# NVlabs/FasterViT

Measured on AMD Instinct MI355X. Metric: images/sec FasterViT-0 224x224 inference, bs=256/GPU, higher is better.
Workload: dtype f16; 1 GPU; faster_vit_0_224 inference, 224x224, batch 256/GPU, synthetic weights (tests/synth.py init family); global_batch=256, parallelism=dp1 (independent shards, no data-path collective), hat_operands=f16, streams=1

## Files before the change

fastervit_amd/csrc/fvit_conv.hip:

```cpp
#include "fvit_common.h"

namespace fvit {

namespace {

constexpr int BK = 64;

struct ConvParams {
    const void* in;
    const void* w;
    const float* bias;
    const void* res;
    void* out;
    const void* zeros;
    int B, Hi, Wi, Cin, Cout, Ho, Wo, stride, act;
    int M, tiles_m, tiles_n;
    int ablate;
    int wterms;
    const void* in_lo;
    const void* res_lo;
    void* out_lo;
    float* out_f32;
    int px;
    int cv, kd;
    float inv_cv;
};

__device__ __forceinline__ int swz_x(int r) { return (r >> 1) & 7; }
__device__ __forceinline__ int swz_w(int r) { return ((0x78 >> (2 * ((r >> 4) & 3))) & 3) | ((r & 2) << 1); }

__device__ __forceinline__ void glds16(const void* gsrc, char* lds_dst) {
    __builtin_amdgcn_global_load_lds((const __attribute__((address_space(1))) void*)gsrc,
                                     (__attribute__((address_space(3))) void*)lds_dst, 16, 0, 0);
}

template <int V> struct IntTag { static constexpr int value = V; };
template <typename F>
__device__ __forceinline__ void dispatch_epilogue(int act, bool has_res, F&& body) {
    if (has_res) {
        if (act == 0) body(IntTag<0>{}, IntTag<1>{});
        else if (act == 1) body(IntTag<1>{}, IntTag<1>{});
        else body(IntTag<2>{}, IntTag<1>{});
    } else {
        if (act == 0) body(IntTag<0>{}, IntTag<0>{});
        else if (act == 1) body(IntTag<1>{}, IntTag<0>{});
        else body(IntTag<2>{}, IntTag<0>{});
    }
}

constexpr int PATCH_H = 8, PATCH_W = 16, PHALO_W = PATCH_W + 2, PHALO_ROWS = (PATCH_H + 2) * PHALO_W;
constexpr int PHALO_PIECES = (PHALO_ROWS + 7) / 8;
constexpr int PHALO_BYTES = PHALO_PIECES * 1024;

template <typename T, int WM, int WN, int NI, bool PX = false, bool DENSE = false, bool HALO = false>
__global__ __launch_bounds__(256, 2) void conv3x3_kernel(ConvParams p) {
    typedef typename Op16<T>::v8 v8;
    static_assert(!HALO || (WM == 2 && WN == 2 && !DENSE), "halo form: 8 x 16 patches on the 2 x 2 wave grid, classic weight layout");
    constexpr int BM = 64 * WM, BN = 16 * NI * WN;
    constexpr int X_BYTES = HALO ? PHALO_BYTES : BM * BK * 2, W_BYTES = BN * BK * 2;
    constexpr int XP = BM / 8 / 4;
    constexpr int HP = (PHALO_PIECES + 3) / 4;
    constexpr int WPIECES = BN / 8;
    constexpr int WP = (WPIECES + 3) / 4;
    static_assert(2 * (X_BYTES + W_BYTES) <= 80 * 1024, "two workgroups per CU");
    __shared__ __attribute__((aligned(16))) char smem[2 * (X_BYTES + W_BYTES)];

    const int tid = threadIdx.x;
    const int lane = tid & 63;
    const int wave = __builtin_amdgcn_readfirstlane(tid >> 6);
    const int wm = wave / WN, wn = wave - wm * WN;

    const int nblk = gridDim.x, b = blockIdx.x;
    const int q = nblk >> 3, rr = nblk & 7, xcd = b & 7, idx = b >> 3;
    const int v = (xcd < rr ? xcd * (q + 1) : rr * (q + 1) + (xcd - rr) * q) + idx;
    const int tm = v / p.tiles_n, tn = v - tm * p.tiles_n;
    const int m0 = tm * BM, n0 = tn * BN;

    const T* __restrict__ In = (const T*)p.in;
    const T* __restrict__ W = (const T*)p.w;
    const T* __restrict__ Z = (const T*)p.zeros;
    const int ldw = DENSE ? p.wterms * p.kd * BK : p.wterms * 9 * p.Cin;

    f4 acc[NI][4];
#pragma unroll
    for (int i = 0; i < NI; ++i)
#pragma unroll
        for (int j = 0; j < 4; ++j) acc[i][j] = (f4){0.f, 0.f, 0.f, 0.f};

    const int g = lane >> 4, s = lane & 15;
    int bimg = 0, y0 = 0, x0 = 0;
    if constexpr (HALO) {
        const int tpx = (p.Wo + PATCH_W - 1) / PATCH_W, tpy = (p.Ho + PATCH_H - 1) / PATCH_H;
        bimg = tm / (tpy * tpx);
        const int rem = tm - bimg * (tpy * tpx);
        const int ty = rem / tpx;
        y0 = ty * PATCH_H;
        x0 = (rem - ty * tpx) * PATCH_W;
    }
    if constexpr (HALO) {
        int hoff[HP];
        int hvalid = 0;
        int hchunk[HP];
#pragma unroll
        for (int i = 0; i < HP; ++i) {
            const int piece = wave + 4 * i;
            const int r = piece * 8 + (lane >> 3);
            const int hy = r / PHALO_W, hx = r - hy * PHALO_W;
            const int iy = y0 - 1 + hy, ix = x0 - 1 + hx;
            const int chunk = ((lane & 7) ^ swz_x(r)) * 8;
            hchunk[i] = chunk;
            const bool ok = piece < PHALO_PIECES && r < PHALO_ROWS && iy >= 0 && iy < p.Hi && ix >= 0 && ix < p.Wi;
            if (ok) hvalid |= 1 << i;
            hoff[i] = ok ? ((bimg * p.Hi + iy) * p.Wi + ix) * p.Cin + chunk : 0;
        }
        const int ncc = p.Cin / BK;
        const int kpb_hi = p.wterms * 9;
        const int nblk_hi = ncc, nblk_all = ncc * ((PX && p.in_lo) ? 2 : 1);
        const int nk = nblk_hi * kpb_hi + (nblk_all - nblk_hi) * 9;
        const T* const InLo = (PX && p.in_lo) ? (const T*)p.in_lo : In;
        auto stage_halo = [&](int blk, char* xbuf) {
            const bool lo = blk >= nblk_hi;
            const T* const plane = lo ? InLo : In;
            const int c0 = (lo ? blk - nblk_hi : blk) * BK;
#pragma unroll
            for (int i = 0; i < HP; ++i) {
                const int piece = wave + 4 * i;
                if (piece < PHALO_PIECES) {
                    const T* src = ((hvalid >> i) & 1) ? plane + (hoff[i] + c0) : Z + hchunk[i];
                    glds16(src, xbuf + piece * 1024);
                }
            }
        };
        auto stage_w = [&](int blk, int kin, char* wbuf) {
            const bool lo = blk >= nblk_hi;
            const int c0 = (lo ? blk - nblk_hi : blk) * BK;
            const int col = kin * p.Cin + c0;
#pragma unroll
            for (int i = 0; i < WP; ++i) {
                const int piece = wave * WP + i;
                if (piece < WPIECES) {
                    const int r = piece * 8 + (lane >> 3);
                    const int c = (lane & 7) ^ swz_w(r);
                    glds16(W + (size_t)min(n0 + r, p.Cout - 1) * ldw + col + c * 8, wbuf + piece * 1024);
                }
            }
        };
        char* const wring = smem + 2 * X_BYTES;
        stage_halo(0, smem);
        stage_w(0, 0, wring);
        int rbase[4], wrow[NI];
#pragma unroll
        for (int i = 0; i < 4; ++i) rbase[i] = (wm * 4 + i) * PHALO_W + s;
#pragma unroll
        for (int i = 0; i < NI; ++i) wrow[i] = wn * 16 * NI + (s >> 2) * 4 * NI + i * 4 + (s & 3);
        int blk = 0, kin = 0, kpb = kpb_hi, hb = 0;
        for (int kt = 0; kt < nk; ++kt) {
            asm volatile("s_waitcnt vmcnt(0)" ::: "memory");
            __syncthreads();
            const int cur = kt & 1;
            int nblk_ = blk, nkin = kin + 1;
            if (nkin == kpb) { nblk_ = blk + 1; nkin = 0; }
            if (kt + 1 < nk) stage_w(nblk_, nkin, wring + (cur ^ 1) * W_BYTES);
            if (kin == 0 && blk + 1 < nblk_all) stage_halo(blk + 1, smem + (hb ^ 1) * X_BYTES);
            const char* xt = smem + hb * X_BYTES;
            const char* wt = wring + cur * W_BYTES;
            const int tap = kin >= 9 ? kin - 9 : kin;
            const int ky = (tap * 11) >> 5, kx = tap - ky * 3;
            const int rsh = ky * PHALO_W + kx;
            v8 xf[2][4], wf[2][NI];
#pragma unroll
            for (int kk = 0; kk < 2; ++kk) {
                const int c = kk * 4 + g;
#pragma unroll
                for (int i = 0; i < 4; ++i) {
                    const int r = rbase[i] + rsh;
                    xf[kk][i] = *(const v8*)(xt + r * 128 + ((c ^ swz_x(r)) << 4));
                }
#pragma unroll
                for (int i = 0; i < NI; ++i) wf[kk][i] = *(const v8*)(wt + wrow[i] * 128 + ((c ^ swz_w(wrow[i])) << 4));
            }
            __builtin_amdgcn_sched_barrier(0);
#pragma unroll
            for (int kk = 0; kk < 2; ++kk)
#pragma unroll
                for (int ni = 0; ni < NI; ++ni)
#pragma unroll
                    for (int mi = 0; mi < 4; ++mi) acc[ni][mi] = Op16<T>::mfma(wf[kk][ni], xf[kk][mi], acc[ni][mi]);
            blk = nblk_; kin = nkin;
            if (kin == 0) { hb ^= 1; kpb = blk >= nblk_hi ? 9 : kpb_hi; }
        }
    } else {
    int64_t rowoff[XP];
    int rowmask[XP];
    int rowchunk[XP];
#pragma unroll
    for (int i = 0; i < XP; ++i) {
        const int r = (wave * XP + i) * 8 + (lane >> 3);
        const int m = m0 + r;
        int mask = 0;
        int64_t base = 0;
        if (m < p.M) {
            const int hw = p.Ho * p.Wo;
            const int bb = m / hw, rem = m - bb * hw;
            const int yo = rem / p.Wo, xo = rem - yo * p.Wo;
            const int yi = yo * p.stride - 1, xi = xo * p.stride - 1;
#pragma unroll
            for (int ky = 0; ky < 3; ++ky)
#pragma unroll
                for (int kx = 0; kx < 3; ++kx)
                    if (yi + ky >= 0 && yi + ky < p.Hi && xi + kx >= 0 && xi + kx < p.Wi) mask |= 1 << (ky * 3 + kx);
            base = (((int64_t)bb * p.Hi + yi) * p.Wi + xi) * p.Cin;
        }
        rowoff[i] = base;
        rowmask[i] = mask;
        rowchunk[i] = ((lane & 7) ^ swz_x(r)) * 8;
    }

    const int cpt = p.Cin / BK;
    const int nk1 = DENSE ? p.kd : 9 * cpt;
    const T* const InLo = (PX && p.in_lo) ? (const T*)p.in_lo : In;
    auto stage_x = [&](int kt, char* xbuf) {
        const int seg = kt >= 2 * nk1 ? 2 : (kt >= nk1 ? 1 : 0);
        const int kta = kt - seg * nk1;
        const T* const plane = (PX && seg == 2) ? InLo : In;
        if constexpr (DENSE) {
            const int k0 = kta * BK;
#pragma unroll
            for (int i = 0; i < XP; ++i) {
                const int k = k0 + rowchunk[i];
                const int tap = (int)(((float)k + 0.5f) * p.inv_cv);
                const int ci = k - tap * p.cv;
                const int ky = (tap * 11) >> 5, kx = tap - ky * 3;
                const int toff = (ky * p.Wi + kx) * p.Cin + ci;
                const T* src = ((rowmask[i] >> tap) & 1) ? plane + (rowoff[i] + toff) : Z + rowchunk[i];
                glds16(src, xbuf + (wave * XP + i) * 1024);
            }
        } else {
        const int tap = kta / cpt, ci0 = (kta - tap * cpt) * BK;
        const int ky = tap / 3, kx = tap - ky * 3;
        const int64_t toff = (ky * p.Wi + kx) * p.Cin + ci0;
        if (!(p.ablate & 1))
#pragma unroll
        for (int i = 0; i < XP; ++i) {
            const T* src = ((rowmask[i] >> tap) & 1) ? plane + (rowoff[i] + toff + rowchunk[i]) : Z + rowchunk[i];
            glds16(src, xbuf + (wave * XP + i) * 1024);
        }
        }
    };
    auto stage_w = [&](int kt, char* wbuf) {
        const int seg = kt >= 2 * nk1 ? 2 : (kt >= nk1 ? 1 : 0);
        const int ktw = seg == 2 ? kt - 2 * nk1 : kt;
        if (!(p.ablate & 2))
#pragma unroll
        for (int i = 0; i < WP; ++i) {
            const int piece = wave * WP + i;
            if (piece < WPIECES) {
                const int r = piece * 8 + (lane >> 3);
                const int c = (lane & 7) ^ swz_w(r);
                glds16(W + (size_t)min(n0 + r, p.Cout - 1) * ldw + ktw * BK + c * 8, wbuf + piece * 1024);
            }
        }
    };

    const int nk = (p.wterms + ((PX && p.in_lo) ? 1 : 0)) * nk1;
    char* const wring = smem + 2 * X_BYTES;
    stage_x(0, smem);
    stage_w(0, wring);

    int xrow[4], wrow[NI];
#pragma unroll
    for (int i = 0; i < 4; ++i) xrow[i] = wm * 64 + i * 16 + s;
#pragma unroll
    for (int i = 0; i < NI; ++i) wrow[i] = wn * 16 * NI + (s >> 2) * 4 * NI + i * 4 + (s & 3);

    for (int kt = 0; kt < nk; ++kt) {
        asm volatile("s_waitcnt vmcnt(0)" ::: "memory");
        __syncthreads();
        const int cur = kt & 1;
        if (kt + 1 < nk) { stage_x(kt + 1, smem + (cur ^ 1) * X_BYTES); stage_w(kt + 1, wring + (cur ^ 1) * W_BYTES); }
        const char* xt = smem + cur * X_BYTES;
        const char* wt = wring + cur * W_BYTES;
        v8 xf[2][4], wf[2][NI];
#pragma unroll
        for (int kk = 0; kk < 2; ++kk) {
            const int c = kk * 4 + g;
#pragma unroll
            for (int i = 0; i < 4; ++i) xf[kk][i] = *(const v8*)(xt + xrow[i] * 128 + ((c ^ swz_x(xrow[i])) << 4));
#pragma unroll
            for (int i = 0; i < NI; ++i) wf[kk][i] = *(const v8*)(wt + wrow[i] * 128 + ((c ^ swz_w(wrow[i])) << 4));
        }
        __builtin_amdgcn_sched_barrier(0);
        if (!(p.ablate & 4))
#pragma unroll
        for (int kk = 0; kk < 2; ++kk)
#pragma unroll
            for (int ni = 0; ni < NI; ++ni)
#pragma unroll
                for (int mi = 0; mi < 4; ++mi) acc[ni][mi] = Op16<T>::mfma(wf[kk][ni], xf[kk][mi], acc[ni][mi]);
    }
    }
    if (p.ablate & 8) return;

    auto rowm = [&](int mi) {
        if constexpr (HALO) {
            const int y = y0 + wm * 4 + mi, x = x0 + s;
            return (y < p.Ho && x < p.Wo) ? (bimg * p.Ho + y) * p.Wo + x : p.M;
        } else {
            return m0 + wm * 64 + mi * 16 + s;
        }
    };
    constexpr int NC = 4 * NI;
    typedef T vout __attribute__((ext_vector_type(NC)));
    const int nb = n0 + wn * 16 * NI + g * NC;
    if (nb >= p.Cout) return;
    float bias[NC];
#pragma unroll
    for (int j = 0; j < NI; ++j) {
        const f4 t = p.bias ? *(const f4*)(p.bias + nb + j * 4) : (f4){0.f, 0.f, 0.f, 0.f};
        bias[j * 4 + 0] = t[0]; bias[j * 4 + 1] = t[1]; bias[j * 4 + 2] = t[2]; bias[j * 4 + 3] = t[3];
    }
    T* O = (T*)p.out;
    const T* R = (const T*)p.res;
    if constexpr (PX) {
        const T* RL = (const T*)p.res_lo;
        T* OL = (T*)p.out_lo;
        float* OF = p.out_f32;
        auto px_epilogue = [&](auto act_tag) {
            constexpr int ACT = decltype(act_tag)::value;
#pragma unroll
            for (int mi = 0; mi < 4; ++mi) {
                const int m = rowm(mi);
                if (m < p.M) {
                    float y[NC];
#pragma unroll
                    for (int ni = 0; ni < NI; ++ni)
#pragma unroll
                        for (int r = 0; r < 4; ++r) {
                            float v = acc[ni][mi][r] + bias[ni * 4 + r];
                            if (ACT == 1) v = fmaxf(v, 0.f);
                            y[ni * 4 + r] = v;
                        }
                    if constexpr (ACT == 2) gelu_erf_each<NC>(y);
                    if (R) {
// ... 925 lines not shown
                const int rc0 = it0 >> 2, rc1 = it1 >> 2;
                const int xa = min(max(x0 + ((it0 & 3) < 3 ? 32 * (it0 & 3) : 66), 0), p.Wi - 1);
                const int xb = min(max(x0 + ((it1 & 3) < 3 ? 32 * (it1 & 3) : 66), 0), p.Wi - 1);
                const int ya = min(max(y0 + rc0 / 3, 0), p.Hi - 1), yb = min(max(y0 + rc1 / 3, 0), p.Hi - 1);
                pf0 = nib[rc0 < 105 ? ((rc0 % 3) * sc + ya * sh + xa * sw) >> 2 : 0];
                pf1 = nib[rc1 < 105 ? ((rc1 % 3) * sc + yb * sh + xb * sw) >> 2 : 0];
            }
            for (int g3 = wave; g3 < SF_GROUPS; g3 += 4 * SF_BATCH) {
                v8 xfb[SF_BATCH];
                int qv[SF_BATCH], lrv[SF_BATCH], lcv[SF_BATCH];
                bool v1v[SF_BATCH];
#pragma unroll
                for (int u = 0; u < SF_BATCH; ++u) {
                    const int q = (g3 + 4 * u) * 16 + lane_s;
                    const int lr = q / SF_COLS, lc = q - lr * SF_COLS;
                    const int R = r0 + (tr ? lc : lr), Cc = c0 + (tr ? lr : lc);
                    const bool v1 = q < SF_ROWS * SF_COLS && R >= 0 && R < p.H1 && Cc >= 0 && Cc < p.W1;
                    const int yi = 2 * R - 1, xi = 2 * Cc - 1;
                    qv[u] = q; lrv[u] = lr; lcv[u] = lc; v1v[u] = v1;
                    unsigned mask = v1 ? m_valid : 0u;
                    if (yi < 0) mask &= ~m_ky0;
                    if (yi + 2 >= p.Hi) mask &= ~m_ky2;
                    if (xi < 0) mask &= ~m_kx0;
                    if (xi + 2 >= p.Wi) mask &= ~m_kx2;
                    const int base = yi * sh + xi * sw;
#pragma unroll
                    for (int e = 0; e < 8; ++e) {
                        const bool inb = (mask >> e) & 1u;
                        const unsigned off = inb ? (unsigned)(base + koff[e]) : 0u;
                        float val = (float)*(const IN*)(ib + off);
                        if constexpr (U8IN) val = __builtin_fmaf(val, nsc3[e % 3], nsh3[e % 3]);
                        xfb[u][e] = (T)(inb ? val : 0.f);
                    }
                }
#pragma unroll
                for (int u = 0; u < SF_BATCH; ++u) {
                    const int q = qv[u], lr = lrv[u], lc = lcv[u];
                    const bool v1 = v1v[u];
                    f4 acc[4];
#pragma unroll
                    for (int ni = 0; ni < 4; ++ni) acc[ni] = Op16<T>::mfma(w1f[ni], xfb[u], (f4){0.f, 0.f, 0.f, 0.f});
                    if (q < SF_ROWS * SF_COLS) {
                        v8 o0, o1;
#pragma unroll
                        for (int ni = 0; ni < 4; ++ni) {
                            const f4 bv = *(const f4*)(sb1 + lane_g * 16 + ni * 4);
#pragma unroll
                            for (int r = 0; r < 4; ++r) {
                                const float y = v1 ? fmaxf(acc[ni][r] + bv[r], 0.f) : 0.f;
                                if (ni < 2) o0[ni * 4 + r] = (T)y; else o1[(ni - 2) * 4 + r] = (T)y;
                            }
                        }
                        const int px = lc >> 1;
                        char* dst = img + lr * SF_ROWPITCH + (lc & 1) * SF_PLANE + px * 128;
                        *(v8*)(dst + (((2 * lane_g) ^ (px & 6)) << 4)) = o0;
                        *(v8*)(dst + (((2 * lane_g + 1) ^ (px & 6)) << 4)) = o1;
                    }
                }
            }
            pf_sink ^= pf0 ^ pf1;
        }
        FVIT_SF_MARK(tsA)
        __syncthreads();
        FVIT_SF_MARK(tsBar)

        const char* hb = img + (2 * ph * 4) * SF_ROWPITCH;
        f4 acc[2][4];
#pragma unroll
        for (int i = 0; i < 2; ++i)
#pragma unroll
            for (int j = 0; j < 4; ++j) acc[i][j] = (f4){0.f, 0.f, 0.f, 0.f};
        v8 xf[2][4];
#pragma unroll
        for (int mi = 0; mi < 4; ++mi) xf[0][mi] = *(const v8*)(hb + (2 * mi) * SF_ROWPITCH + xoff[0]);
        __builtin_amdgcn_sched_barrier(0);
        static_assert(SF_ROWPITCH % 256 == 0, "a row shift must leave bit 6 of a read offset alone");
        int ko[2][3];
#pragma unroll
        for (int k = 0; k < 3; ++k) {
            ko[0][k] = tr ? xoff[k] : k * SF_ROWPITCH;
            ko[1][k] = tr ? k * SF_ROWPITCH : xoff[k];
        }
#pragma unroll
        for (int q = 0; q < 18; ++q) {
            const int tap = q >> 1, kk = q & 1;
            if (q + 1 < 18) {
                const int tap1 = (q + 1) >> 1, kk1 = (q + 1) & 1, ky1 = tap1 / 3, kx1 = tap1 - ky1 * 3;
                const int o = (ko[0][ky1] + ko[1][kx1]) ^ (kk1 << 6);
#pragma unroll
                for (int mi = 0; mi < 4; ++mi) xf[(q + 1) & 1][mi] = *(const v8*)(hb + (2 * mi) * SF_ROWPITCH + o);
            }
#pragma unroll
            for (int ni = 0; ni < 2; ++ni)
#pragma unroll
                for (int mi = 0; mi < 4; ++mi) acc[ni][mi] = Op16<T>::mfma(wf[tap][kk][ni], xf[q & 1][mi], acc[ni][mi]);
            __builtin_amdgcn_sched_barrier(0);
        }

        FVIT_SF_MARK(tsB)
        const f4 t0 = *(const f4*)(sb2 + nb), t1 = *(const f4*)(sb2 + nb + 4);
        const float bias[8] = {t0[0], t0[1], t0[2], t0[3], t1[0], t1[1], t1[2], t1[3]};
#pragma unroll
        for (int mi = 0; mi < 4; ++mi) {
            const int row = ph * 4 + mi;
            const int y = tp.y0 + (tr ? s : row), x = tp.x0 + (tr ? row : s);
            if (y < p.H2 && x < p.W2) {
                v8 ov;
#pragma unroll
                for (int ni = 0; ni < 2; ++ni)
#pragma unroll
                    for (int r = 0; r < 4; ++r) ov[ni * 4 + r] = (T)fmaxf(acc[ni][mi][r] + bias[ni * 4 + r], 0.f);
                *(v8*)(O + (((size_t)b * p.H2 + y) * p.W2 + x) * 64 + nb) = ov;
            }
        }
        FVIT_SF_MARK(tsE)
    }
    if (pf_sink == 0x9E3779B1u && p.tiles == -12345) ((unsigned*)p.out)[0] = pf_sink;
    if constexpr (TS) {
        if (p.ts && lane == 0) {
            unsigned long long* o = p.ts + ((size_t)blockIdx.x * 4 + wave) * 8;
            o[0] = tsA; o[1] = tsBar; o[2] = tsB; o[3] = tsE; o[4] = tsBar0; o[5] = tsN; o[6] = __builtin_amdgcn_s_memtime() - tsT0; o[7] = 0;
        }
    }
#undef FVIT_SF_MARK
}

enum ConvRoute : int {
    CR_NONE = -1,
    CR_HALO64, CR_HALO64_LN,
    CR_BAND128, CR_BAND128_LN,
    CR_PATCH, CR_PATCH_PX,
    CR_T128, CR_T128_DENSE, CR_T128_PX, CR_T128_PX_DENSE,
    CR_T64, CR_T64_DENSE, CR_T64_PX, CR_T64_PX_DENSE,
    CR_T256X64,
    CR_COUNT
};
struct ConvRouteInfo { const char* name; int bm, bn; };
constexpr ConvRouteInfo kConvRoutes[CR_COUNT] = {
    {"conv3x3_c64_halo_kernel", 0, 0},         {"conv3x3_c64_halo_kernel<ln>", 0, 0},
    {"conv3x3_c128_band_kernel", 0, 0},        {"conv3x3_c128_band_kernel<ln>", 0, 0},
    {"conv3x3_kernel<2,2,4,patch>", 128, 128}, {"conv3x3_kernel<2,2,4,px,patch>", 128, 128},
    {"conv3x3_kernel<2,2,4>", 128, 128},       {"conv3x3_kernel<2,2,4,dense>", 128, 128},
    {"conv3x3_kernel<2,2,4,px>", 128, 128},    {"conv3x3_kernel<2,2,4,px,dense>", 128, 128},
    {"conv3x3_kernel<2,2,2>", 128, 64},        {"conv3x3_kernel<2,2,2,dense>", 128, 64},
    {"conv3x3_kernel<2,2,2,px>", 128, 64},     {"conv3x3_kernel<2,2,2,px,dense>", 128, 64},
    {"conv3x3_kernel<4,1,4>", 256, 64},
};
inline bool route_is_ln(int r) { return r == CR_HALO64_LN || r == CR_BAND128_LN; }

struct ConvKnobs {
    int halo = tune_get("conv_halo", 1), band = tune_get("conv_band", 1);
    int patch = tune_get("conv_patch", 1), patch_max_waste_pct = tune_get("conv_patch_max_waste_pct", 10);
    int n128_ragged = tune_get("conv_n128_ragged", 1), narrow = tune_get("conv128_narrow", 0), variant64 = tune_get("conv64_variant", 0);
};

inline int out_size(int n, int stride) { return (n + 2 - 3) / stride + 1; }
inline bool call_is_px(const FvitConvCall& c) { return c.px || c.in_lo || c.residual_lo || c.out_lo || c.out_f32; }

int validate_conv(const char* who, int32_t dtype, const FvitConvWeights* w, const FvitConvCall* c) {
    if (!w || !c) { set_error("%s: null weights or call", who); return FVIT_EINVAL; }
    const bool px = call_is_px(*c);
    if (!c->in || !(w->classic || w->dense || w->band_frag) || (!c->out && !c->out_f32) || !c->zeros || c->B <= 0 || c->Hi <= 0 || c->Wi <= 0 ||
        c->Cin <= 0 || c->Cout <= 0 || (c->Cin % 64) || (c->Cout % 64) || (c->stride != 1 && c->stride != 2) || c->act < 0 || c->act > 2 ||
        (w->terms != 1 && w->terms != 2) || (c->in_lo && w->terms != 2) || (c->residual_lo && !c->residual) || (c->out_f32 && c->out_lo) ||
        (c->out_lo && !c->out)) {
        set_error("%s: unsupported arguments Cin=%d Cout=%d stride=%d act=%d weight_terms=%d (need Cin %% 64 == 0, Cout %% 64 == 0, stride 1|2, "
                  "weight_terms 2 with a two-term input, out or out_f32)", who, c->Cin, c->Cout, c->stride, c->act, w->terms);
        return FVIT_EINVAL;
    }
    if (w->cin_valid != c->Cin && (w->cin_valid <= 0 || w->cin_valid > c->Cin || (w->cin_valid % 8))) {
        set_error("%s: cin_valid=%d must be a multiple of 8 in (0, Cin=%d]", who, w->cin_valid, c->Cin);
        return FVIT_EINVAL;
    }
    const int64_t M = (int64_t)c->B * out_size(c->Hi, c->stride) * out_size(c->Wi, c->stride);
    if (M > 0x7fffffff) {
        set_error("%s: %lld output pixels exceed the 32-bit row index", who, (long long)M);
        return FVIT_EINVAL;
    }
    if (c->ln_w && (!c->ln_b || !c->residual || c->stride != 1 || c->act != 0 || px)) {
        set_error("%s: the LayerNorm2d epilogue needs ln_w and ln_b, a residual, stride 1, no activation and 16-bit maps", who);
        return FVIT_EINVAL;
    }
    if (dtype != FVIT_F16 && dtype != FVIT_BF16) {
        set_error("%s: dtype %d not supported (16-bit %s only)", who, dtype, px ? "planes" : "maps");
        return FVIT_EINVAL;
    }
    return FVIT_OK;
}

ConvRoute choose_conv_route(const FvitConvCall& c, const FvitConvWeights& w, const ConvKnobs& k) {
    const int Ho = out_size(c.Hi, c.stride), Wo = out_size(c.Wi, c.stride);
    const int64_t M = (int64_t)c.B * Ho * Wo;
    const bool px = call_is_px(c), ln = c.ln_w != nullptr;
    const bool padded = w.cin_valid != c.Cin;
    const bool plain16 = c.stride == 1 && w.terms == 1 && !px && !padded;
    if (c.Cin == 64 && c.Cout == 64 && plain16 && w.classic && k.halo)
        return ln && M * 64 <= 0x7fffffff ? CR_HALO64_LN : CR_HALO64;
    if (c.Cin == 128 && c.Cout == 128 && plain16 && w.band_frag && k.band && band_supported(c.Hi, c.Wi) && M * 128 <= 0x7fffffff)
        return ln ? CR_BAND128_LN : CR_BAND128;
    const bool n128 = c.Cout % 128 == 0 || (c.Cout > 128 && k.n128_ragged);
    if (w.classic && k.patch && c.stride == 1 && c.Cout >= 128 && n128 && !k.narrow && (int64_t)c.B * c.Hi * c.Wi * c.Cin < 0x7fffffffLL) {
        const int64_t tiles = (int64_t)c.B * ((Ho + PATCH_H - 1) / PATCH_H) * ((Wo + PATCH_W - 1) / PATCH_W);
        if (tiles * 128 * 100 <= M * (100 + k.patch_max_waste_pct)) return px ? CR_PATCH_PX : CR_PATCH;
    }
    const bool dense = padded && w.dense;
    if (!dense && !w.classic) {
        set_error("conv3x3: no kernel for Cin=%d Cout=%d stride=%d on a %d x %d map reads the weight images given (classic%s rows needed)", c.Cin, c.Cout,
                  c.stride, c.Hi, c.Wi, padded ? " or dense" : "");
        return CR_NONE;
    }
    if (px) return ConvRoute((n128 ? CR_T128_PX : CR_T64_PX) + dense);
    if (n128 && !k.narrow) return ConvRoute(CR_T128 + dense);
    return k.variant64 == 1 && !dense ? CR_T256X64 : ConvRoute(CR_T64 + dense);
}

using ConvKernel = void (*)(ConvParams);
template <typename T>
ConvKernel gemm_kernel(ConvRoute r) {
    switch (r) {
    case CR_PATCH: return conv3x3_kernel<T, 2, 2, 4, false, false, true>;
    case CR_PATCH_PX: return conv3x3_kernel<T, 2, 2, 4, true, false, true>;
    case CR_T128: return conv3x3_kernel<T, 2, 2, 4, false, false>;
    case CR_T128_DENSE: return conv3x3_kernel<T, 2, 2, 4, false, true>;
    case CR_T128_PX: return conv3x3_kernel<T, 2, 2, 4, true, false>;
    case CR_T128_PX_DENSE: return conv3x3_kernel<T, 2, 2, 4, true, true>;
    case CR_T64: return conv3x3_kernel<T, 2, 2, 2, false, false>;
    case CR_T64_DENSE: return conv3x3_kernel<T, 2, 2, 2, false, true>;
    case CR_T64_PX: return conv3x3_kernel<T, 2, 2, 2, true, false>;
    case CR_T64_PX_DENSE: return conv3x3_kernel<T, 2, 2, 2, true, true>;
    default: return conv3x3_kernel<T, 4, 1, 4>;
    }
}

template <typename T>
int run_conv(ConvRoute r, const FvitConvCall& c, const FvitConvWeights& w, hipStream_t stream, void* stamps = nullptr) {
    const char* name = kConvRoutes[r].name;
    const int Ho = out_size(c.Hi, c.stride), Wo = out_size(c.Wi, c.stride), M = c.B * Ho * Wo;
    const bool ln = route_is_ln(r);
    if (r == CR_HALO64 || r == CR_HALO64_LN) {
        if (ablate_skip(64)) return FVIT_OK;
        HaloParams p;
        p.ln_w = ln ? c.ln_w : nullptr; p.ln_b = c.ln_b; p.ln_eps = c.ln_eps;
        p.in = c.in; p.w = w.classic; p.bias = c.bias; p.res = c.residual; p.out = c.out; p.zeros = c.zeros;
        p.B = c.B; p.H = c.Hi; p.W = c.Wi; p.act = c.act;
        const EdgeTiling et = edge_tiling(c.Hi, c.Wi, c.act != 2 && tune_get("conv_edge_tiles", 1));
        p.tiles_x = et.tiles_x; p.tiles_y = et.tiles_y; p.strips = et.strips;
        p.tiles = c.B * (p.tiles_x * p.tiles_y + p.strips);
        p.ablate = diag_knob("conv_halo_ablate");
        int maxgrid = tune_get("conv_halo_grid", 512);
        if (maxgrid < 8) maxgrid = 8;
        const EdgeTiling pt = edge_tiling(c.Hi, c.Wi, 0);
        const int plain_tiles = c.B * pt.tiles_x * pt.tiles_y;
        const int grid = plain_tiles < maxgrid ? plain_tiles : maxgrid;
        ProfScope prof(FVIT_K_CONV, 2.0 * M * 64.0 * 576.0, 2.0 * ((double)M * 64 * (c.residual ? 3.0 : 2.0) + 576.0 * 64), stream);
        prof_note(name, grid);
        p.buf_bytes = c.residual ? HALO_BUF : HALO_BYTES;
        const void* kern = ln ? (const void*)conv3x3_c64_halo_kernel<T, true> : (const void*)conv3x3_c64_halo_kernel<T>;
        const size_t lds = ln ? HALO_LN_LDS : 1024 + 2 * (size_t)p.buf_bytes;
        static DeviceOnce once[2];
        if (once[ln].first_on_current_device()) hipFuncSetAttribute(kern, hipFuncAttributeMaxDynamicSharedMemorySize, ln ? HALO_LN_LDS : 1024 + 2 * HALO_BUF);
        if (tune_get("conv_halo_debug", 0)) {
            int nb = -1;
            hipOccupancyMaxActiveBlocksPerMultiprocessor(&nb, kern, 256, lds);
            fprintf(stderr, "[fvit] %s: grid %d, tiles %d, dynamic LDS %zu B, resident workgroups/CU %d\n", name, grid, p.tiles, lds, nb);
        }
        if (ln) hipLaunchKernelGGL((conv3x3_c64_halo_kernel<T, true>), dim3(grid), dim3(256), lds, stream, p);
        else hipLaunchKernelGGL((conv3x3_c64_halo_kernel<T>), dim3(grid), dim3(256), lds, stream, p);
        return check_launch(name);
    }
    if (ablate_skip(32)) return FVIT_OK;
    if (r == CR_BAND128 || r == CR_BAND128_LN) {
        BandParams p;
        p.in = c.in; p.wf = w.band_frag; p.bias = c.bias; p.res = c.residual; p.out = c.out; p.zeros = c.zeros;
        p.B = c.B; p.H = c.Hi; p.W = c.Wi; p.act = c.act;
        p.ln_w = ln ? c.ln_w : nullptr; p.ln_b = c.ln_b; p.ln_eps = c.ln_eps;
        p.PW = c.Wi + 2;
        p.R = (BD_NG * 16) / p.PW;
        if (p.R > c.Hi) p.R = c.Hi;
        p.bands = (c.Hi + p.R - 1) / p.R;
        p.npieces = ((p.R + 2) * p.PW + 3) / 4;
        p.magic = (65536 + p.PW - 1) / p.PW;
        p.ts = (unsigned long long*)stamps;
        const dim3 grid(c.B * p.bands);
        ProfScope prof(FVIT_K_CONV, 2.0 * M * 128.0 * 1152.0, 2.0 * ((double)M * 128 * (c.residual ? 3.0 : 2.0) + 1152.0 * 128), stream);
        prof_note(name, c.B * p.bands);
        if (ln) hipLaunchKernelGGL((conv3x3_c128_band_kernel<T, false, true>), grid, dim3(256), 0, stream, p);
        else if (std::is_same<T, _Float16>::value && stamps) hipLaunchKernelGGL((conv3x3_c128_band_kernel<_Float16, true>), grid, dim3(256), 0, stream, p);
        else hipLaunchKernelGGL((conv3x3_c128_band_kernel<T>), grid, dim3(256), 0, stream, p);
        return check_launch(name);
    }
    const bool px = call_is_px(c), dense = r >= CR_T128 && ((r - CR_T128) & 1), patch = r == CR_PATCH || r == CR_PATCH_PX;
    ConvParams p;
    p.in = c.in; p.w = dense ? w.dense : w.classic; p.bias = c.bias; p.res = c.residual; p.out = c.out; p.zeros = c.zeros;
    p.B = c.B; p.Hi = c.Hi; p.Wi = c.Wi; p.Cin = c.Cin; p.Cout = c.Cout; p.Ho = Ho; p.Wo = Wo; p.stride = c.stride; p.act = c.act; p.M = M;
    p.ablate = px ? 0 : diag_knob("conv_ablate"); p.wterms = w.terms;
    p.in_lo = c.in_lo; p.res_lo = c.residual_lo; p.out_lo = c.out_lo; p.out_f32 = c.out_f32; p.px = px;
    p.cv = dense ? w.cin_valid : 0; p.kd = dense ? (9 * p.cv + BK - 1) / BK : 0; p.inv_cv = dense ? 1.0f / (float)p.cv : 0.f;
    p.tiles_m = patch ? c.B * ((Ho + PATCH_H - 1) / PATCH_H) * ((Wo + PATCH_W - 1) / PATCH_W) : (M + kConvRoutes[r].bm - 1) / kConvRoutes[r].bm;
    p.tiles_n = (c.Cout + kConvRoutes[r].bn - 1) / kConvRoutes[r].bn;
    const double flops = 2.0 * M * (double)c.Cout * 9.0 * (dense ? p.cv : c.Cin);
    const double bytes = 2.0 * ((double)c.B * c.Hi * c.Wi * c.Cin * (c.in_lo ? 2.0 : 1.0) +
                                (double)M * c.Cout * ((c.residual ? (c.residual_lo ? 2.0 : 1.0) : 0.0) + ((c.out_lo || c.out_f32) ? 2.0 : 1.0)) + 9.0 * w.terms * c.Cin * c.Cout);
    ProfScope prof(FVIT_K_CONV, flops, bytes, stream);
    prof_note(name, p.tiles_m * p.tiles_n);
    hipLaunchKernelGGL(gemm_kernel<T>(r), dim3(p.tiles_m * p.tiles_n), dim3(256), 0, stream, p);
    return check_launch(name);
}

int launch_route(int32_t dtype, ConvRoute r, const FvitConvCall& c, const FvitConvWeights& w, fvit_stream_t stream, void* stamps = nullptr) {
    return dtype == FVIT_F16 ? run_conv<_Float16>(r, c, w, (hipStream_t)stream, stamps) : run_conv<__bf16>(r, c, w, (hipStream_t)stream, stamps);
}

int conv_entry(int32_t dtype, const FvitConvWeights* w, const FvitConvCall* c, bool run, fvit_stream_t stream) {
    const char* who = c && call_is_px(*c) ? "conv3x3_px" : "conv3x3";
    if (const int rc = validate_conv(who, dtype, w, c)) return rc;
    const ConvRoute r = choose_conv_route(*c, *w, ConvKnobs{});
    if (r == CR_NONE) return FVIT_EINVAL;
    if (!run) return r;
    if (c->ln_w && !route_is_ln(r)) {
        set_error("%s: %s has no LayerNorm2d epilogue (ask fvit_conv3x3_route first and run the LayerNorm2d pass apart)", who, kConvRoutes[r].name);
        return FVIT_EINVAL;
    }
    return launch_route(dtype, r, *c, *w, stream);
}

FvitConvCall one_call(const void* in, const float* bias, const void* residual, void* out, const void* zeros, int B, int Hi, int Wi, int Cin, int Cout,
                      int stride, int act) {
    FvitConvCall c{};
    c.in = in; c.bias = bias; c.residual = residual; c.out = out; c.zeros = zeros;
    c.B = B; c.Hi = Hi; c.Wi = Wi; c.Cin = Cin; c.Cout = Cout; c.stride = stride; c.act = act;
    return c;
}
int one_image_conv(int32_t dtype, FvitConvCall c, const void* weight, int cin_valid, int terms, fvit_stream_t stream) {
    FvitConvWeights w{};
    (cin_valid == c.Cin ? w.classic : w.dense) = weight;
    w.terms = terms; w.cin_valid = cin_valid;
    return conv_entry(dtype, &w, &c, true, stream);
}
static_assert(BD_MAXPW == 32, "the W <= 30 in the messages of the row-band entry points");
int named_conv(const char* who, const char* need, int32_t dtype, FvitConvCall c, const void* classic, const void* band_frag, ConvRoute want, const float* ln_w,
               const float* ln_b, float eps, fvit_stream_t stream, void* stamps = nullptr) {
    const FvitConvWeights w{classic, nullptr, band_frag, 1, c.Cin};
    c.ln_w = ln_w; c.ln_b = ln_b; c.ln_eps = eps;
    ConvKnobs k;
    k.halo = k.band = 1;
    if (validate_conv(who, dtype, &w, &c) == FVIT_OK && choose_conv_route(c, w, k) == want) return launch_route(dtype, want, c, w, stream, stamps);
    if (dtype == FVIT_F16 || dtype == FVIT_BF16) set_error("%s: unsupported arguments B=%d H=%d W=%d act=%d (need %s)", who, c.B, c.Hi, c.Wi, c.act, need);
    return FVIT_EINVAL;
}

}
}

using namespace fvit;

extern "C" int fvit_conv3x3(int32_t dtype, const FvitConvWeights* weights, const FvitConvCall* call, fvit_stream_t stream) { return conv_entry(dtype, weights, call, true, stream); }

extern "C" int fvit_conv3x3_route(int32_t dtype, const FvitConvWeights* weights, const FvitConvCall* call) { return conv_entry(dtype, weights, call, false, nullptr); }

extern "C" const char* fvit_conv3x3_route_name(int route) { return route >= 0 && route < CR_COUNT ? kConvRoutes[route].name : "?"; }

extern "C" int fvit_conv3x3_dense_k(int32_t cin_valid) { return cin_valid > 0 && cin_valid % 8 == 0 ? (9 * cin_valid + BK - 1) / BK * BK : -1; }

extern "C" int fvit_conv3x3_nhwc(int32_t dtype, const void* in, const void* weight, const float* bias, const void* residual, void* out,
                                 int32_t B, int32_t Hi, int32_t Wi, int32_t Cin, int32_t Cout, int32_t stride, int32_t act,
                                 const void* zeros, fvit_stream_t stream) {
    return one_image_conv(dtype, one_call(in, bias, residual, out, zeros, B, Hi, Wi, Cin, Cout, stride, act), weight, Cin, 1, stream);
}

extern "C" int fvit_conv3x3_nhwc_terms(int32_t dtype, const void* in, const void* weight, const float* bias, const void* residual, void* out,
                                       int32_t B, int32_t Hi, int32_t Wi, int32_t Cin, int32_t Cout, int32_t stride, int32_t act,
                                       int32_t weight_terms, const void* zeros, fvit_stream_t stream) {
    return one_image_conv(dtype, one_call(in, bias, residual, out, zeros, B, Hi, Wi, Cin, Cout, stride, act), weight, Cin, weight_terms, stream);
}

extern "C" int fvit_conv3x3_nhwc_dense(int32_t dtype, const void* in, const void* weight, const float* bias, const void* residual, void* out,
                                       int32_t B, int32_t Hi, int32_t Wi, int32_t Cin, int32_t cin_valid, int32_t Cout, int32_t stride, int32_t act,
                                       int32_t weight_terms, const void* zeros, fvit_stream_t stream) {
    return one_image_conv(dtype, one_call(in, bias, residual, out, zeros, B, Hi, Wi, Cin, Cout, stride, act), weight, cin_valid, weight_terms, stream);
}

extern "C" int fvit_conv3x3_nhwc_px_dense(int32_t dtype, const void* in, const void* in_lo, const void* weight, const float* bias, const void* residual,
                                          const void* residual_lo, void* out, void* out_lo, float* out_f32, int32_t B, int32_t Hi, int32_t Wi, int32_t Cin,
                                          int32_t cin_valid, int32_t Cout, int32_t stride, int32_t act, int32_t weight_terms, const void* zeros,
                                          fvit_stream_t stream) {
    FvitConvCall c = one_call(in, bias, residual, out, zeros, B, Hi, Wi, Cin, Cout, stride, act);
    c.in_lo = in_lo; c.residual_lo = residual_lo; c.out_lo = out_lo; c.out_f32 = out_f32; c.px = 1;
    return one_image_conv(dtype, c, weight, cin_valid, weight_terms, stream);
}

extern "C" int fvit_conv3x3_nhwc_px(int32_t dtype, const void* in, const void* in_lo, const void* weight, const float* bias, const void* residual,
                                    const void* residual_lo, void* out, void* out_lo, float* out_f32, int32_t B, int32_t Hi, int32_t Wi, int32_t Cin,
                                    int32_t Cout, int32_t stride, int32_t act, int32_t weight_terms, const void* zeros, fvit_stream_t stream) {
    return fvit_conv3x3_nhwc_px_dense(dtype, in, in_lo, weight, bias, residual, residual_lo, out, out_lo, out_f32, B, Hi, Wi, Cin, Cin, Cout, stride, act,
                                      weight_terms, zeros, stream);
}

extern "C" int fvit_conv3x3_patch_form(int32_t B, int32_t Hi, int32_t Wi, int32_t Cin, int32_t Cout, int32_t stride) {
    const FvitConvWeights w{&w, nullptr, nullptr, 2, Cin};
    const FvitConvCall c = one_call(&w, nullptr, nullptr, (void*)&w, &w, B, Hi, Wi, Cin, Cout, stride, 0);
    return conv_entry(FVIT_F16, &w, &c, false, nullptr) == CR_PATCH ? 1 : 0;
}

extern "C" int fvit_conv3x3_c128_band_supported(int32_t H, int32_t W) {
    const FvitConvWeights w{nullptr, nullptr, &w, 1, 128};
    const FvitConvCall c = one_call(&w, nullptr, nullptr, (void*)&w, &w, 1, H, W, 128, 128, 1, 0);
    return conv_entry(FVIT_F16, &w, &c, false, nullptr) == CR_BAND128 ? 1 : 0;
}

extern "C" int fvit_conv3x3_c128_band(int32_t dtype, const void* in, const void* w_frag, const float* bias, const void* residual, void* out,
                                      int32_t B, int32_t H, int32_t W, int32_t act, const void* zeros, fvit_stream_t stream) {
    return named_conv("conv3x3_c128_band", "W <= 30", dtype, one_call(in, bias, residual, out, zeros, B, H, W, 128, 128, 1, act), nullptr, w_frag, CR_BAND128,
                      nullptr, nullptr, 0.f, stream);
}

extern "C" int fvit_conv3x3_c64_ln2d(int32_t dtype, const void* in, const void* weight, const float* bias, const void* residual, void* out,
                                     const float* ln_w, const float* ln_b, float eps, int32_t B, int32_t H, int32_t W, const void* zeros,
                                     fvit_stream_t stream) {
    return named_conv("conv3x3_c64_ln2d", "a residual and LayerNorm2d parameters", dtype, one_call(in, bias, residual, out, zeros, B, H, W, 64, 64, 1, 0), weight,
                      nullptr, CR_HALO64_LN, ln_w, ln_b, eps, stream);
}

extern "C" int fvit_conv3x3_c128_band_ln2d(int32_t dtype, const void* in, const void* w_frag, const float* bias, const void* residual, void* out,
                                           const float* ln_w, const float* ln_b, float eps, int32_t B, int32_t H, int32_t W, const void* zeros,
                                           fvit_stream_t stream) {
    return named_conv("conv3x3_c128_band_ln2d", "a residual, LayerNorm2d parameters and W <= 30", dtype,
                      one_call(in, bias, residual, out, zeros, B, H, W, 128, 128, 1, 0), nullptr, w_frag, CR_BAND128_LN, ln_w, ln_b, eps, stream);
}

#ifdef FVIT_DIAG
extern "C" int fvit_debug_conv_band_timeline(const void* in, const void* w_frag, const float* bias, const void* residual, void* out, int32_t B,
                                             int32_t H, int32_t W, int32_t act, const void* zeros, void* stamps, fvit_stream_t stream) {
    if (!stamps) { set_error("debug_conv_band_timeline: null stamp buffer"); return FVIT_EINVAL; }
    return named_conv("debug_conv_band_timeline", "W <= 30", FVIT_F16, one_call(in, bias, residual, out, zeros, B, H, W, 128, 128, 1, act), nullptr, w_frag,
                      CR_BAND128, nullptr, nullptr, 0.f, stream, stamps);
}
#endif

static bool stem_image_type_ok(const char* entry, const FvitMapView* in, const float* norm, bool u8_entry) {
    if (!u8_entry && in->dtype == FVIT_U8) {
        set_error("%s: a uint8 (FVIT_U8) image needs its normalisation constants: call %s_u8", entry, entry);
        return false;
    }
    if (u8_entry && in->dtype != FVIT_U8) {
        set_error("%s_u8: image dtype %d is not FVIT_U8: call %s", entry, in->dtype, entry);
        return false;
    }
    if (u8_entry && !norm) {
        set_error("%s_u8: null normalisation constants", entry);
        return false;
    }
    return true;
}

static int stem_conv_impl(const char* entry, int32_t dtype, const FvitMapView* in, const void* weight, const void* weight_lo, const float* bias, void* out,
                          int32_t B, int32_t Hi, int32_t Wi, fvit_stream_t stream, const float* norm, bool u8_entry);

extern "C" int fvit_stem_conv3x3s2(int32_t dtype, const FvitMapView* in, const void* weight, const float* bias, void* out, int32_t B,
                                   int32_t Hi, int32_t Wi, fvit_stream_t stream) {
    return stem_conv_impl("fvit_stem_conv3x3s2", dtype, in, weight, nullptr, bias, out, B, Hi, Wi, stream, nullptr, false);
}

extern "C" int fvit_stem_conv3x3s2_px(int32_t dtype, const FvitMapView* in, const void* weight, const void* weight_lo, const float* bias, void* out,
                                      int32_t B, int32_t Hi, int32_t Wi, fvit_stream_t stream) {
    return stem_conv_impl("fvit_stem_conv3x3s2_px", dtype, in, weight, weight_lo, bias, out, B, Hi, Wi, stream, nullptr, false);
}

extern "C" int fvit_stem_conv3x3s2_u8(int32_t dtype, const FvitMapView* in, const void* weight, const float* bias, void* out, int32_t B,
                                      int32_t Hi, int32_t Wi, fvit_stream_t stream, const float* norm) {
    return stem_conv_impl("fvit_stem_conv3x3s2", dtype, in, weight, nullptr, bias, out, B, Hi, Wi, stream, norm, true);
}

extern "C" int fvit_stem_conv3x3s2_px_u8(int32_t dtype, const FvitMapView* in, const void* weight, const void* weight_lo, const float* bias, void* out,
                                         int32_t B, int32_t Hi, int32_t Wi, fvit_stream_t stream, const float* norm) {
    return stem_conv_impl("fvit_stem_conv3x3s2_px", dtype, in, weight, weight_lo, bias, out, B, Hi, Wi, stream, norm, true);
}

static int stem_conv_impl(const char* entry, int32_t dtype, const FvitMapView* in, const void* weight, const void* weight_lo, const float* bias, void* out,
                          int32_t B, int32_t Hi, int32_t Wi, fvit_stream_t stream, const float* norm, bool u8_entry) {
    if (!in || !in->data || !weight || !bias || !out || B <= 0 || Hi <= 0 || Wi <= 0) {
        set_error("stem_conv: null or empty argument");
        return FVIT_EINVAL;
    }
    if (!stem_image_type_ok(entry, in, norm, u8_entry)) return FVIT_EINVAL;
    const bool u8 = u8_entry;
    StemParams p;
    for (int c = 0; c < 3; ++c) { p.nscale[c] = u8 ? norm[c] : 1.f; p.nshift[c] = u8 ? norm[3 + c] : 0.f; }
    p.in = *in; p.w = weight; p.w_lo = weight_lo; p.bias = bias; p.out = out; p.B = B; p.Hi = Hi; p.Wi = Wi;
    p.Ho = (Hi - 1) / 2 + 1;
    p.Wo = (Wi - 1) / 2 + 1;
    const int64_t M = (int64_t)B * p.Ho * p.Wo;
    if (M > 0x7fffffff) {
        set_error("stem_conv: too many output pixels");
        return FVIT_EINVAL;
    }
    p.M = (int)M;
    const int nblk16 = (p.M + 15) / 16;
    int grid = (nblk16 + 3) / 4;
    if (grid > 256 * 32) grid = 256 * 32;
// ... 119 lines not shown
```

Measured before the change: 97770 images/s.

## Add five-slot operand ring pipeline for plain 128x128 conv3x3 kernel

Adds a KPIPE variant of the 128x128 implicit-GEMM conv3x3 kernel. It streams X and W k-tiles through a five-slot LDS ring, with split requests, explicit vmcnt waits and interleaved LDS reads and MFMAs, so global loads overlap compute across k-steps. The variant is enabled by default via a conv_kpipe knob for the CR_T128 route. This adds hand-tuned scheduling complexity and only applies where the plain T128 route is chosen; for FasterViT-0 most convs likely take the patch or halo routes instead.

```diff
diff --git a/fastervit_amd/csrc/fvit_conv.hip b/fastervit_amd/csrc/fvit_conv.hip
--- a/fastervit_amd/csrc/fvit_conv.hip
+++ b/fastervit_amd/csrc/fvit_conv.hip
@@ -52,18 +52,27 @@
 constexpr int PHALO_PIECES = (PHALO_ROWS + 7) / 8;
 constexpr int PHALO_BYTES = PHALO_PIECES * 1024;
 
-template <typename T, int WM, int WN, int NI, bool PX = false, bool DENSE = false, bool HALO = false>
+constexpr int KP_SLOTS = 5, KP_UNIT = 128 * BK * 2;
+__device__ __forceinline__ void kp_wait(int n) {
+    if (n == 8) asm volatile("s_waitcnt vmcnt(8)" ::: "memory");
+    else if (n == 4) asm volatile("s_waitcnt vmcnt(4)" ::: "memory");
+    else asm volatile("s_waitcnt vmcnt(0)" ::: "memory");
+}
+
+template <typename T, int WM, int WN, int NI, bool PX = false, bool DENSE = false, bool HALO = false, bool KPIPE = false>
 __global__ __launch_bounds__(256, 2) void conv3x3_kernel(ConvParams p) {
     typedef typename Op16<T>::v8 v8;
     static_assert(!HALO || (WM == 2 && WN == 2 && !DENSE), "halo form: 8 x 16 patches on the 2 x 2 wave grid, classic weight layout");
+    static_assert(!KPIPE || (WM == 2 && WN == 2 && NI == 4 && !PX && !DENSE && !HALO), "operand ring: the plain 128 x 128 instance");
     constexpr int BM = 64 * WM, BN = 16 * NI * WN;
     constexpr int X_BYTES = HALO ? PHALO_BYTES : BM * BK * 2, W_BYTES = BN * BK * 2;
     constexpr int XP = BM / 8 / 4;
     constexpr int HP = (PHALO_PIECES + 3) / 4;
     constexpr int WPIECES = BN / 8;
     constexpr int WP = (WPIECES + 3) / 4;
-    static_assert(2 * (X_BYTES + W_BYTES) <= 80 * 1024, "two workgroups per CU");
-    __shared__ __attribute__((aligned(16))) char smem[2 * (X_BYTES + W_BYTES)];
+    constexpr int SMEM_BYTES = KPIPE ? KP_SLOTS * KP_UNIT : 2 * (X_BYTES + W_BYTES);
+    static_assert(SMEM_BYTES <= 80 * 1024, "two workgroups per CU");
+    __shared__ __attribute__((aligned(16))) char smem[SMEM_BYTES];
 
     const int tid = threadIdx.x;
     const int lane = tid & 63;
@@ -189,6 +198,115 @@
             blk = nblk_; kin = nkin;
             if (kin == 0) { hb ^= 1; kpb = blk >= nblk_hi ? 9 : kpb_hi; }
         }
+    } else if constexpr (KPIPE) {
+#ifdef FVIT_DIAG
+        const int ablate = p.ablate;
+#else
+        constexpr int ablate = 0;
+#endif
+        const int rqx = (ablate & 1) ? 0 : 4, rqw = (ablate & 2) ? 0 : 4;
+        int64_t xsrc[4];
+        int rowmask[4];
+        int zchunk[4];
+        size_t wsrc[4];
+#pragma unroll
+        for (int i = 0; i < 4; ++i) {
+            const int r = (wave * 4 + i) * 8 + (lane >> 3);
+            const int m = m0 + r;
+            int mask = 0;
+            int64_t base = 0;
+            if (m < p.M) {
+                const int hw = p.Ho * p.Wo;
+                const int bb = m / hw, rem = m - bb * hw;
+                const int yo = rem / p.Wo, xo = rem - yo * p.Wo;
+                const int yi = yo * p.stride - 1, xi = xo * p.stride - 1;
+#pragma unroll
+                for (int ky = 0; ky < 3; ++ky)
+#pragma unroll
+                    for (int kx = 0; kx < 3; ++kx)
+                        if (yi + ky >= 0 && yi + ky < p.Hi && xi + kx >= 0 && xi + kx < p.Wi) mask |= 1 << (ky * 3 + kx);
+                base = (((int64_t)bb * p.Hi + yi) * p.Wi + xi) * p.Cin;
+            }
+            zchunk[i] = ((lane & 7) ^ swz_x(r)) * 8;
+            xsrc[i] = base + zchunk[i];
+            rowmask[i] = mask;
+            wsrc[i] = (size_t)min(n0 + r, p.Cout - 1) * ldw + ((lane & 7) ^ swz_w(r)) * 8;
+        }
+        const int nk = p.wterms * 9 * (p.Cin / BK);
+        int rt = 0, rc = 0, rw = 0;
+        auto request_x = [&](char* slot) {
+            const int ky = (rt * 11) >> 5, kx = rt - ky * 3;
+            const int64_t toff = (ky * p.Wi + kx) * p.Cin + rc;
+            if (!(ablate & 1))
+#pragma unroll
+                for (int i = 0; i < 4; ++i) {
+                    const T* src = ((rowmask[i] >> rt) & 1) ? In + (xsrc[i] + toff) : Z + zchunk[i];
+                    glds16(src, slot + (wave * 4 + i) * 1024);
+                }
+            rc += BK;
+            if (rc == p.Cin) { rc = 0; rt = rt == 8 ? 0 : rt + 1; }
+        };
+        auto request_w = [&](char* slot) {
+            if (!(ablate & 2))
+#pragma unroll
+                for (int i = 0; i < 4; ++i) glds16(W + (wsrc[i] + (size_t)rw * BK), slot + (wave * 4 + i) * 1024);
+            ++rw;
+        };
+        const int xbase = (wm * 64 + s) * 128, wbase = (wn * 64 + (s >> 2) * 16 + (s & 3)) * 128;
+        const int xsw = swz_x(wm * 64 + s), wsw = swz_w(wn * 64 + (s >> 2) * 16 + (s & 3));
+        const int xfo[2] = {xbase + ((g ^ xsw) << 4), xbase + (((4 + g) ^ xsw) << 4)};
+        const int wfo[2] = {wbase + ((g ^ wsw) << 4), wbase + (((4 + g) ^ wsw) << 4)};
+        auto read = [&](const char* xu, const char* wu, int kk, v8 (&xf)[4], v8 (&wf)[4]) {
+#pragma unroll
+            for (int i = 0; i < 4; ++i) {
+                xf[i] = *(const v8*)(xu + xfo[kk] + i * 2048);
+                wf[i] = *(const v8*)(wu + wfo[kk] + i * 512);
+            }
+        };
+        auto mfma_half = [&](v8 (&xc)[4], v8 (&wc)[4], bool reads) {
+            if (!(ablate & 4))
+#pragma unroll
+                for (int ni = 0; ni < 4; ++ni)
+#pragma unroll
+                    for (int mi = 0; mi < 4; ++mi) acc[ni][mi] = Op16<T>::mfma(wc[ni], xc[mi], acc[ni][mi]);
+            if (reads) {
+#pragma unroll
+                for (int j = 0; j < 8; ++j) {
+                    __builtin_amdgcn_sched_group_barrier(0x008, 1, 0);
+                    __builtin_amdgcn_sched_group_barrier(0x100, 1, 0);
+                }
+                __builtin_amdgcn_sched_group_barrier(0x008, 8, 0);
+            }
+            __builtin_amdgcn_sched_barrier(0);
+        };
+        auto slot = [&](int u) { return smem + (u >= KP_SLOTS ? u - KP_SLOTS : u) * KP_UNIT; };
+        int su = 0;
+        v8 xa[4], wa[4], xb[4], wb[4];
+        auto kstep = [&](auto req_tag, auto next_tag) {
+            constexpr bool REQ = decltype(req_tag)::value != 0;
+            constexpr int NEXT = decltype(next_tag)::value;
+            if constexpr (REQ) request_x(slot(su + 4));
+            __builtin_amdgcn_sched_barrier(0);
+            read(slot(su), slot(su + 1), 1, xb, wb);
+            mfma_half(xa, wa, true);
+            if constexpr (NEXT) {
+                if (NEXT == 1) kp_wait(rqx); else kp_wait(0);
+                asm volatile("s_waitcnt lgkmcnt(0)\n\ts_barrier" ::: "memory");
+                if constexpr (REQ) request_w(slot(su));
+                __builtin_amdgcn_sched_barrier(0);
+                read(slot(su + 2), slot(su + 3), 0, xa, wa);
+            }
+            mfma_half(xb, wb, NEXT != 0);
+            su = su + 2 >= KP_SLOTS ? su + 2 - KP_SLOTS : su + 2;
+        };
+        request_x(slot(0)); request_w(slot(1)); request_x(slot(2)); request_w(slot(3));
+        kp_wait(rqx + rqw);
+        asm volatile("s_barrier" ::: "memory");
+        read(slot(0), slot(1), 0, xa, wa);
+        __builtin_amdgcn_sched_barrier(0);
+        for (int kt = 0; kt < nk - 2; ++kt) kstep(IntTag<1>{}, IntTag<1>{});
+        kstep(IntTag<0>{}, IntTag<2>{});
+        kstep(IntTag<0>{}, IntTag<0>{});
     } else {
     int64_t rowoff[XP];
     int rowmask[XP];
@@ -1420,6 +1538,7 @@
     int halo = tune_get("conv_halo", 1), band = tune_get("conv_band", 1);
     int patch = tune_get("conv_patch", 1), patch_max_waste_pct = tune_get("conv_patch_max_waste_pct", 10);
     int n128_ragged = tune_get("conv_n128_ragged", 1), narrow = tune_get("conv128_narrow", 0), variant64 = tune_get("conv64_variant", 0);
+    int kpipe = tune_get("conv_kpipe", 1);
 };
 
 inline int out_size(int n, int stride) { return (n + 2 - 3) / stride + 1; }
@@ -1484,11 +1603,11 @@
 
 using ConvKernel = void (*)(ConvParams);
 template <typename T>
-ConvKernel gemm_kernel(ConvRoute r) {
+ConvKernel gemm_kernel(ConvRoute r, bool kpipe) {
     switch (r) {
     case CR_PATCH: return conv3x3_kernel<T, 2, 2, 4, false, false, true>;
     case CR_PATCH_PX: return conv3x3_kernel<T, 2, 2, 4, true, false, true>;
-    case CR_T128: return conv3x3_kernel<T, 2, 2, 4, false, false>;
+    case CR_T128: return kpipe ? conv3x3_kernel<T, 2, 2, 4, false, false, false, true> : conv3x3_kernel<T, 2, 2, 4, false, false>;
     case CR_T128_DENSE: return conv3x3_kernel<T, 2, 2, 4, false, true>;
     case CR_T128_PX: return conv3x3_kernel<T, 2, 2, 4, true, false>;
     case CR_T128_PX_DENSE: return conv3x3_kernel<T, 2, 2, 4, true, true>;
@@ -1501,7 +1620,7 @@
 }
 
 template <typename T>
-int run_conv(ConvRoute r, const FvitConvCall& c, const FvitConvWeights& w, hipStream_t stream, void* stamps = nullptr) {
+int run_conv(ConvRoute r, const FvitConvCall& c, const FvitConvWeights& w, const ConvKnobs& k, hipStream_t stream, void* stamps = nullptr) {
     const char* name = kConvRoutes[r].name;
     const int Ho = out_size(c.Hi, c.stride), Wo = out_size(c.Wi, c.stride), M = c.B * Ho * Wo;
     const bool ln = route_is_ln(r);
@@ -1571,25 +1690,26 @@
                                 (double)M * c.Cout * ((c.residual ? (c.residual_lo ? 2.0 : 1.0) : 0.0) + ((c.out_lo || c.out_f32) ? 2.0 : 1.0)) + 9.0 * w.terms * c.Cin * c.Cout);
     ProfScope prof(FVIT_K_CONV, flops, bytes, stream);
     prof_note(name, p.tiles_m * p.tiles_n);
-    hipLaunchKernelGGL(gemm_kernel<T>(r), dim3(p.tiles_m * p.tiles_n), dim3(256), 0, stream, p);
+    hipLaunchKernelGGL(gemm_kernel<T>(r, k.kpipe != 0), dim3(p.tiles_m * p.tiles_n), dim3(256), 0, stream, p);
     return check_launch(name);
 }
 
-int launch_route(int32_t dtype, ConvRoute r, const FvitConvCall& c, const FvitConvWeights& w, fvit_stream_t stream, void* stamps = nullptr) {
-    return dtype == FVIT_F16 ? run_conv<_Float16>(r, c, w, (hipStream_t)stream, stamps) : run_conv<__bf16>(r, c, w, (hipStream_t)stream, stamps);
+int launch_route(int32_t dtype, ConvRoute r, const FvitConvCall& c, const FvitConvWeights& w, const ConvKnobs& k, fvit_stream_t stream, void* stamps = nullptr) {
+    return dtype == FVIT_F16 ? run_conv<_Float16>(r, c, w, k, (hipStream_t)stream, stamps) : run_conv<__bf16>(r, c, w, k, (hipStream_t)stream, stamps);
 }
 
 int conv_entry(int32_t dtype, const FvitConvWeights* w, const FvitConvCall* c, bool run, fvit_stream_t stream) {
     const char* who = c && call_is_px(*c) ? "conv3x3_px" : "conv3x3";
     if (const int rc = validate_conv(who, dtype, w, c)) return rc;
-    const ConvRoute r = choose_conv_route(*c, *w, ConvKnobs{});
+    const ConvKnobs k;
+    const ConvRoute r = choose_conv_route(*c, *w, k);
     if (r == CR_NONE) return FVIT_EINVAL;
     if (!run) return r;
     if (c->ln_w && !route_is_ln(r)) {
         set_error("%s: %s has no LayerNorm2d epilogue (ask fvit_conv3x3_route first and run the LayerNorm2d pass apart)", who, kConvRoutes[r].name);
         return FVIT_EINVAL;
     }
-    return launch_route(dtype, r, *c, *w, stream);
+    return launch_route(dtype, r, *c, *w, k, stream);
 }
 
 FvitConvCall one_call(const void* in, const float* bias, const void* residual, void* out, const void* zeros, int B, int Hi, int Wi, int Cin, int Cout,
@@ -1612,7 +1732,7 @@
     c.ln_w = ln_w; c.ln_b = ln_b; c.ln_eps = eps;
     ConvKnobs k;
     k.halo = k.band = 1;
-    if (validate_conv(who, dtype, &w, &c) == FVIT_OK && choose_conv_route(c, w, k) == want) return launch_route(dtype, want, c, w, stream, stamps);
+    if (validate_conv(who, dtype, &w, &c) == FVIT_OK && choose_conv_route(c, w, k) == want) return launch_route(dtype, want, c, w, k, stream, stamps);
     if (dtype == FVIT_F16 || dtype == FVIT_BF16) set_error("%s: unsupported arguments B=%d H=%d W=%d act=%d (need %s)", who, c.B, c.Hi, c.Wi, c.act, need);
     return FVIT_EINVAL;
 }
```

Measured after the change: 96520 images/s. -1.3%, worse.
